# therealadityashankar/hey-buddy

Hardware: AMD Instinct MI355X
Metric: audio clips/sec featurized+trained, 1.5 s @16 kHz, 1/2/4/8 GPU (higher is better)
Workload: dtype f32

## Files before the change

### hey-buddy_amd/csrc/hbk_clip_ops.hip

```cpp
#include <algorithm>

#include "hbk_aug_dev.h"

namespace hbk {
namespace {

struct TanhArgs {
  const float* x;
  int64_t x_stride;
  float* out;
  int64_t out_stride;
  int64_t n_clips;
  const float* amount;
  const int32_t* idx;
  int64_t n_entries;
  SrcView view;
};

__device__ __forceinline__ unsigned abs_bits(float v, int s) {
  return s < kT ? (__builtin_bit_cast(unsigned, v) & 0x7FFFFFFFu) : 0xFFFFFFFFu;
}

__global__ void __launch_bounds__(kThreads) __attribute__((amdgpu_waves_per_eu(8)))
tanh_distortion_kernel(TanhArgs a) {
  __shared__ unsigned hist[4096];
  __shared__ float red[32];
  __shared__ unsigned pick[2];
  constexpr int kPer = (kT + kThreads - 1) / kThreads;
  const int64_t n_iter = a.idx ? a.n_entries : a.n_clips;
  for (int64_t e = blockIdx.x; e < n_iter; e += gridDim.x) {
    const int64_t clip = a.idx ? a.idx[e] : e;
    const int tid = opaque_tid();
    const float* x = a.x + clip * a.x_stride;
    float* out = a.out + clip * a.out_stride;
    const float amt = a.amount[clip];
    if (amt != amt) {
      if (out != x) copy_clip(x, out, tid);
      continue;
    }
    float xr[kPer];
    const int pre = a.view.pre ? a.view.pre[clip] : -1, len = a.view.pre ? a.view.len[clip] : 0;
    if (pre >= 0) {
      const int n = min(len, kT);
      const float* row = n > 0 ? a.view.src + clip * a.view.stride : x;
      const int t = opaque_tid();
      const int w0 = __builtin_amdgcn_readfirstlane(t & ~63);
#pragma unroll
      for (int u = 0; u < kPer; ++u) xr[u] = load_placed_wave(row, pre, n, w0 + u * kThreads, t & 63);
    } else {
    const int t = opaque_tid();
#pragma unroll
    for (int u = 0; u < kPer; ++u) {
      const int s = t + u * kThreads;
      xr[u] = s < kT ? *reinterpret_cast<const float*>(reinterpret_cast<const char*>(x) + (static_cast<uint32_t>(s) << 2))
                     : 0.f;
    }
    }
    const double pos = (100.0 - 99.0 * static_cast<double>(amt)) / 100.0 * (kT - 1);
    const int lo = min(max(static_cast<int>(floor(pos)), 0), kT - 1);
    const double frac = pos - lo;
    unsigned prefix = 0, mask = 0, rank = static_cast<unsigned>(lo);
#pragma unroll 1
    for (int p = 0; p < 3; ++p) {
      const int shift = p == 0 ? 19 : (p == 1 ? 9 : 0), bins = p == 0 ? 4096 : (p == 1 ? 1024 : 512);
      const int per_lane = bins >> 6;
      for (int i = tid; i < bins; i += kThreads) hist[i] = 0;
      __syncthreads();
      const int t = opaque_tid();
#pragma unroll
      for (int u = 0; u < kPer; ++u) {
        const unsigned b = abs_bits(xr[u], t + u * kThreads);
        if ((b & mask) == prefix && b != 0xFFFFFFFFu) atomicAdd(&hist[(b >> shift) & (bins - 1)], 1u);
      }
      __syncthreads();
      if (tid < 64) {
        unsigned own = 0;
        for (int i = 0; i < per_lane; ++i) own += hist[per_lane * tid + i];
        unsigned inc = own;
#pragma unroll
        for (int d = 1; d < 64; d <<= 1) {
          const unsigned v = __shfl_up(inc, d, 64);
          if (tid >= d) inc += v;
        }
        const unsigned long long hit = __ballot(inc > rank);
        const int l = __ffsll(static_cast<long long>(hit)) - 1;
        if (tid == l) {
          unsigned r = rank - (inc - own), dsel = per_lane * l;
          for (int i = 0; i < per_lane - 1; ++i) {
            const unsigned h = hist[dsel];
            if (r < h) break;
            r -= h;
            ++dsel;
          }
          pick[0] = dsel;
          pick[1] = r;
        }
      }
      __syncthreads();
      prefix |= pick[0] << shift;
      mask |= static_cast<unsigned>(bins - 1) << shift;
      rank = pick[1];
    }
    float cnt = 0.f, mg = __builtin_inff();
    const int t2 = opaque_tid();
#pragma unroll
    for (int u = 0; u < kPer; ++u) {
      const unsigned b = abs_bits(xr[u], t2 + u * kThreads);
      if (b == 0xFFFFFFFFu) continue;
      if (b <= prefix) cnt += 1.f;
      else mg = fminf(mg, __builtin_bit_cast(float, b));
    }
    cnt = block_sum(cnt, red);
    {
      for (int d = 32; d >= 1; d >>= 1) mg = fminf(mg, __shfl_xor(mg, d, 64));
      __syncthreads();
      if ((tid & 63) == 0) red[tid >> 6] = mg;
      __syncthreads();
      mg = red[0];
      for (int w = 1; w < kThreads / 64; ++w) mg = fminf(mg, red[w]);
    }
    const double v_lo = __builtin_bit_cast(float, prefix);
    const double v_hi = (cnt >= lo + 2 || lo + 1 >= kT) ? v_lo : static_cast<double>(mg);
    const double d = v_hi - v_lo;
    const double th = frac >= 0.5 ? v_hi - d * (1.0 - frac) : v_lo + d * frac;
    const float g = static_cast<float>(0.5 / (th + 1e-6));
    float ex = 0.f, ey = 0.f;
#pragma unroll
    for (int u = 0; u < kPer; ++u) {
      ex += xr[u] * xr[u];
      xr[u] = 1.f - __fdividef(2.f, __expf(2.f * g * xr[u]) + 1.f);
      ey += xr[u] * xr[u];
    }
    block_sum2(ex, ey, red);
    const float rms_x = sqrtf(ex / kT);
    const float post = rms_x > 1e-9f ? rms_x / sqrtf(ey / kT) : 1.f;
    const int t3 = opaque_tid();
#pragma unroll
    for (int u = 0; u < kPer; ++u) {
      const int s = t3 + u * kThreads;
      if (s < kT) *reinterpret_cast<float*>(reinterpret_cast<char*>(out) + (static_cast<uint32_t>(s) << 2)) = xr[u] * post;
    }
    __syncthreads();
  }
}

constexpr int kPlaceSpan = 4096;
__global__ void __launch_bounds__(256) place_kernel(const float* __restrict__ src, int64_t src_stride,
                                                    const int32_t* __restrict__ src_len,
                                                    const int32_t* __restrict__ pre,
                                                    const int32_t* __restrict__ idx, float* __restrict__ out,
                                                    int64_t out_stride, int64_t n_clips, int T) {
  const int spans = (T + kPlaceSpan - 1) / kPlaceSpan;
  const int64_t items = n_clips * spans;
  constexpr int kR = kPlaceSpan / 1024;
  for (int64_t it = blockIdx.x; it < items; it += gridDim.x) {
    const int64_t e = it / spans;
    const int sp = static_cast<int>(it - e * spans);
    const int64_t clip = idx ? idx[e] : e;
    const int p = pre[clip];
    const int n = min(src_len[clip], T);
    const int last = max(n - 1, 0);
    const float* s = src + clip * src_stride;
    float* o = out + clip * out_stride;
    const int t0 = sp * kPlaceSpan + 4 * static_cast<int>(threadIdx.x);
    float v[kR][4];
#pragma unroll
    for (int r = 0; r < kR; ++r)
#pragma unroll
      for (int q = 0; q < 4; ++q) {
        const int u = t0 + r * 1024 + q - p;
        const float x = n > 0 ? s[min(max(u, 0), last)] : 0.f;
        v[r][q] = (u >= 0 && u < n) ? x : 0.f;
      }
#pragma unroll
    for (int r = 0; r < kR; ++r) {
      const int t = t0 + r * 1024;
      if (t < T) *reinterpret_cast<float4*>(o + t) = make_float4(v[r][0], v[r][1], v[r][2], v[r][3]);
    }
  }
}

constexpr int kEqTile = 64;
struct EqArgs {
  const float* x;
  int64_t x_stride;
  const double* coef;
  const int32_t* idx;
  float* out;
  int64_t out_stride;
  int64_t n;
  SrcView view;
};

constexpr int kEqClips = 8;
__global__ void __launch_bounds__(64) eq_kernel(EqArgs a) {
  constexpr int kRow = kEqTile + 4;
  __shared__ __attribute__((aligned(16))) float tin[kEqClips][kRow];
  __shared__ __attribute__((aligned(16))) float tout[kEqClips][kRow];
  const int lane = threadIdx.x, c = lane >> 3, sec = lane & 7;
  const int64_t j0 = static_cast<int64_t>(blockIdx.x) * kEqClips;
  const int64_t jc = min(j0 + c, a.n - 1);
  const double* cf0 = a.coef + jc * 35;
  const bool copy = cf0[0] != cf0[0];
  const int k = min(sec, 6);
  double b0 = cf0[5 * k], b1 = cf0[5 * k + 1], b2 = cf0[5 * k + 2], a1 = cf0[5 * k + 3], a2 = cf0[5 * k + 4];
  if (copy) b0 = 1.0, b1 = b2 = a1 = a2 = 0.0;
  double s1 = 0.0, s2 = 0.0;
  const int lc = lane >> 3, lq = lane & 7;
  const int64_t jl = min(j0 + lc, a.n - 1);
  const int64_t clip_l = a.idx ? static_cast<int64_t>(a.idx[jl]) : jl;
  const float* xl = a.x + clip_l * a.x_stride;
  float* ol = a.out + clip_l * a.out_stride;
  const bool store_l = j0 + lc < a.n;
  const int pre_l = a.view.pre ? a.view.pre[clip_l] : -1, len_l = a.view.pre ? a.view.len[clip_l] : 0;
  const int n_l = pre_l >= 0 ? min(len_l, kT) : 0;
  const float* sl = n_l > 0 ? a.view.src + clip_l * a.view.stride : xl;
  float4 p0, p1;
  auto load_tile = [&](int t) {
    const int u0 = t + 4 * lq - pre_l;
    if (pre_l >= 0 && u0 >= 0 && u0 + 35 < n_l) {
      const float* q = sl + u0;
      p0 = float4{q[0], q[1], q[2], q[3]};
      p1 = float4{q[32], q[33], q[34], q[35]};
    } else if (pre_l >= 0 && (u0 + 35 < 0 || u0 >= n_l)) {
      p0 = p1 = float4{0.f, 0.f, 0.f, 0.f};
    } else if (pre_l >= 0) {
// ... 158 lines not shown
```

### hey-buddy_amd/csrc/hbk_embed.hip

```cpp
#include <algorithm>
#include <cmath>
#include <cstring>
#include <numeric>
#include <vector>

#include "hbk_common.h"
#include "hbk_embed_args.h"
#include "hbk_embed_plan.h"

namespace hbk {
namespace {

constexpr int kWaves = kThreads / 64;
constexpr int kChunkClips = 16384;
inline int64_t chunk_clips() {
  static const int64_t c = [] {
    const char* e = getenv("HBK_EMBED_CHUNK");
    const long long v = e ? atoll(e) : 0;
    return v >= 256 && v <= 32768 ? int64_t(v) : int64_t(kChunkClips);
  }();
  return c;
}

typedef float f4 __attribute__((ext_vector_type(4)));

template <int NB, int RB, bool WG>
__device__ __forceinline__ void conv_stage(const float* __restrict__ X, float* __restrict__ Y,
                                           const float* __restrict__ Wst,
                                           const int* __restrict__ ktab,
                                           const float* __restrict__ bias, int G, int hin, int win,
                                           const StageDesc& S, int wstride, int lane, int wave) {
  const int ho = hin - S.kh + 1, wo = win - S.kw + 1;
  const int img_pos = ho * wo, M = G * img_pos;
  const int nrb = (M + 15) >> 4;
  const int r16 = lane & 15, kq = lane >> 4;
  const int nblk = (S.cout + 15) >> 4;
  for (int cb = 0; cb < nblk; cb += NB)
  for (int rb0 = wave * RB; rb0 < nrb; rb0 += kWaves * RB) {
    int moff[RB];
#pragma unroll
    for (int r = 0; r < RB; ++r) {
      int m = min((rb0 + r) * 16 + r16, M - 1);
      const int g = m / img_pos;
      const int rem = m - g * img_pos;
      const int y = rem / wo;
      const int x = rem - y * wo;
      moff[r] = ((g * hin + y) * win + x) * S.cinp;
    }
    f4 acc[RB][NB];
#pragma unroll
    for (int r = 0; r < RB; ++r)
#pragma unroll
      for (int c = 0; c < NB; ++c) acc[r][c] = f4{0.f, 0.f, 0.f, 0.f};
    const float* wp = Wst + kq * wstride + cb * 16 + r16;
#pragma unroll 2
    for (int ks = 0; ks < S.ksteps; ++ks) {
      const int koff = ktab[ks * 4 + kq];
      float av[RB], bv[NB];
#pragma unroll
      for (int r = 0; r < RB; ++r) av[r] = X[moff[r] + koff];
#pragma unroll
      for (int c = 0; c < NB; ++c) bv[c] = wp[ks * 4 * wstride + min(c, nblk - 1 - cb) * 16];
#pragma unroll
      for (int r = 0; r < RB; ++r)
#pragma unroll
        for (int c = 0; c < NB; ++c)
          acc[r][c] = __builtin_amdgcn_mfma_f32_16x16x4f32(av[r], bv[c], acc[r][c], 0, 0, 0);
    }
#pragma unroll
    for (int c = 0; c < NB; ++c) {
      const int n = (cb + c) * 16 + r16;
      if (n >= S.cout) continue;
      const float bb = bias[n];
#pragma unroll
      for (int r = 0; r < RB; ++r)
#pragma unroll
        for (int i = 0; i < 4; ++i) {
          const int m = (rb0 + r) * 16 + kq * 4 + i;
          if (m < M) {
            float v = acc[r][c][i] + bb;
            if (S.act) v = v >= 0.f ? v : v * S.alpha;
            Y[m * S.coutp + n] = v;
          }
        }
    }
  }
  (void)WG;
}

template <int NB, int RB, bool WG>
__global__ void __launch_bounds__(kThreads) conv_chain_kernel(ChainArgs a) {
  extern __shared__ __attribute__((aligned(16))) float smem[];
  float* X = smem + a.lds_x;
  float* Y = smem + a.lds_y;
  float* Wl = smem + a.lds_w;
  int* ktab = reinterpret_cast<int*>(smem + a.lds_k);
  const int tid = threadIdx.x, lane = tid & 63, wave = tid >> 6;
  if (!WG)
    for (int i = tid; i < a.wblob_floats; i += kThreads) Wl[i] = a.wblob[i];

  const int64_t n_groups = (a.n_img + a.G - 1) / a.G;
  const int64_t n_tasks = n_groups * a.n_bands;
  const int C = a.C_src;
  const int cinp0 = a.st[0].cinp;
  for (int64_t task = blockIdx.x; task < n_tasks; task += gridDim.x) {
    const int64_t grp = task / a.n_bands;
    const int band = static_cast<int>(task - grp * a.n_bands);
    const int64_t img0 = grp * a.G;
    const int G = static_cast<int>(min<int64_t>(a.G, a.n_img - img0));
    const int orow0 = band * a.band;
    const int orows = min(a.band, a.H_out - orow0);
    const int r0 = orow0 * a.out_ph;
    const int rows_in = orows * a.out_ph + a.shrink;

    const int row_elems = a.W_in * C;
    const int per_img = rows_in * row_elems;
    for (int e = tid; e < G * per_img; e += kThreads) {
      const int g = e / per_img;
      int rem = e - g * per_img;
      const int r = rem / row_elems;
      rem -= r * row_elems;
      const int w = rem / C;
      const int c = rem - w * C;
      const int64_t im = img0 + g;
      const int64_t clip = im / a.ipc;
      const int roff = a.row_off[im - clip * a.ipc];
      const float* src = a.in + clip * a.src_clip_stride +
                         static_cast<int64_t>(roff + (r0 + r) * a.in_ph) * a.src_row_stride +
                         (w * a.in_pw) * C + c;
      float v = src[0];
      for (int i = 0; i < a.in_ph; ++i)
        for (int j = 0; j < a.in_pw; ++j) v = nan_max(v, src[i * a.src_row_stride + j * C]);
      X[((g * rows_in + r) * a.W_in + w) * cinp0 + c] = v;
    }

    int hin = rows_in, win = a.W_in;
    float* cur = X;
    float* nxt = Y;
    for (int s = 0; s < a.n_stages; ++s) {
      const StageDesc S = a.st[s];
      __syncthreads();
      for (int k = tid; k < S.ksteps * 4; k += kThreads) {
        int v = 0;
        if (k < S.K) {
          const int tap = k / S.cin;
          const int ci = k - tap * S.cin;
          const int dh = tap / S.kw;
          const int dw = tap - dh * S.kw;
          v = (dh * win + dw) * S.cinp + ci;
        }
        ktab[k] = v;
      }
      __syncthreads();
      const float* Wst = WG ? a.wblob + S.w_off : Wl + S.w_off;
      conv_stage<NB, RB, WG>(cur, nxt, Wst, ktab, a.wblob + S.b_off, G, hin, win, S, a.wstride,
                             lane, wave);
      float* t = cur;
      cur = nxt;
      nxt = t;
      hin -= S.kh - 1;
      win -= S.kw - 1;
    }
    __syncthreads();

    const int coutp = a.st[a.n_stages - 1].coutp;
    const int orow_elems = a.W_out * a.C_out;
    const int per_out = orows * orow_elems;
    for (int e = tid; e < G * per_out; e += kThreads) {
      const int g = e / per_out;
      int rem = e - g * per_out;
      const int r = rem / orow_elems;
      rem -= r * orow_elems;
      const int w = rem / a.C_out;
      const int c = rem - w * a.C_out;
      const float* p = cur + ((g * hin + r * a.out_ph) * win + w * a.out_pw) * coutp + c;
// ... 1892 lines not shown
    case Kern::p1s: return f ? addr(p1s_chain_kernel<true>) : addr(p1s_chain_kernel<false>);
    case Kern::p2s: return f ? addr(p2s_chain_kernel<true>) : addr(p2s_chain_kernel<false>);
    case Kern::t3s: return f ? addr(t3s_chain_kernel<true>) : addr(t3s_chain_kernel<false>);
  }
  return nullptr;
}

hipError_t set_max_dynamic_lds(const void* fn) {
  hipFuncAttributes at;
  hipError_t e = hipFuncGetAttributes(&at, fn);
  if (e != hipSuccess) return e;
  return hipFuncSetAttribute(fn, hipFuncAttributeMaxDynamicSharedMemorySize,
                             int(160 * 1024 - static_cast<int>(at.sharedSizeBytes)));
}

void set_pointers(ChainArgs& a, const Launch&, const unsigned char* blob) {
  a.wblob = reinterpret_cast<const float*>(blob);
}
void set_pointers(XArgs& x, const Launch& L, const unsigned char* blob) {
  x.wblob = reinterpret_cast<const _Float16*>(blob);
  x.bblob = reinterpret_cast<const float*>(blob + L.ptr_off[1]);
  x.ktab = reinterpret_cast<const int*>(blob + L.ptr_off[2]);
  x.i2c_off = reinterpret_cast<const int*>(blob + L.ptr_off[3]);
}
template <class A>
void set_pointers(A& p, const Launch& L, const unsigned char* blob) {
  p.w = reinterpret_cast<const _Float16*>(blob);
  if (L.ptr_off[1] >= L.blob.size()) return;
  const float* bias = reinterpret_cast<const float*>(blob + L.ptr_off[1]);
  if constexpr (std::is_same_v<A, P2sArgs>) p.bias_a = bias;
  else p.bias = bias;
}

int realise(const Launch& L, bool pattern, bool debug, Slot& s) {
  const void* fn = kernel_address(L.kernel);
  hipError_t e = hipMalloc(&s.d_blob, L.blob.size());
  if (e != hipSuccess && !pattern) return hip_error(e, "hipMalloc chain weights");
  if (e == hipSuccess) e = hipMemcpy(s.d_blob, L.blob.data(), L.blob.size(), hipMemcpyHostToDevice);
  if (e != hipSuccess && !pattern) return hip_error(e, "copy chain weights");
  if (pattern) {
    if (e == hipSuccess) e = hipFuncSetAttribute(fn, hipFuncAttributeMaxDynamicSharedMemorySize, int(L.lds_bytes));
    if (e == hipSuccess) e = hipOccupancyMaxActiveBlocksPerMultiprocessor(&s.blocks_per_cu, fn, L.threads, L.lds_bytes);
    if (e != hipSuccess || s.blocks_per_cu < 1) {
      (void)hipGetLastError();
      if (s.d_blob) (void)hipFree(s.d_blob);
      s.d_blob = nullptr;
      return HBK_OK;
    }
  } else {
    if (L.lds_bytes > 64 * 1024) {
      e = set_max_dynamic_lds(fn);
      if (e != hipSuccess) return hip_error(e, "hipFuncSetAttribute(max dynamic LDS)");
    }
    s.blocks_per_cu = L.kernel.kind == Kern::exact
                          ? 2
                          : std::max<int>(1, std::min<int>(4, int((160 * 1024) / std::max<size_t>(L.lds_bytes, 1))));
  }
  s.plan = &L;
  s.fn = fn;
  s.args = L.args;
  std::visit([&](auto& a) { set_pointers(a, L, static_cast<const unsigned char*>(s.d_blob)); }, s.args);
  if (debug && pattern) fprintf(stderr, "%s, %d blocks/CU\n", L.debug.c_str(), s.blocks_per_cu);
  if (debug && !pattern) fputs(L.debug.c_str(), stderr);
  return HBK_OK;
}

int realise_program(const ProgramPlan& prog, bool debug, std::vector<ChainPlan>& dev) {
  dev.resize(prog.chains.size());
  for (size_t k = 0; k < dev.size(); ++k) {
    const int rc = realise(prog.chains[k].base, false, debug, dev[k].base);
    if (rc) return rc;
    if (prog.chains[k].pattern) realise(*prog.chains[k].pattern, true, debug, dev[k].pattern);
  }
  return HBK_OK;
}

void bind(ChainArgs& a, const float* in, int64_t stride, float* out, int64_t n_img, int*) {
  a.in = in;
  a.src_clip_stride = stride;
  a.out = out;
  a.n_img = n_img;
}
void bind(XArgs& x, const float* in, int64_t stride, float* out, int64_t n_img, int* range_flag) {
  x.range_flag = range_flag;
  x.in = in;
  x.src_clip_stride = stride;
  x.out = out;
  if ((reinterpret_cast<uintptr_t>(x.out) & 15) || (x.out_img_stride & 3)) x.vec_out = 0;
  if ((reinterpret_cast<uintptr_t>(x.in) & 15) || (x.src_clip_stride & 3) || (x.src_row_stride & 3)) x.raw_vec = 0;
  x.n_img = n_img;
}
template <class A>
void bind(A& p, const float* in, int64_t stride, float* out, int64_t n_img, int* range_flag) {
  p.range_flag = range_flag;
  p.in = in;
  if constexpr (std::is_same_v<A, T3sArgs>) p.src_clip_stride = stride;
  else p.src_img_stride = stride;
  p.out = out;
  p.n_img = n_img;
}

int run_program(const ProgramPlan& prog, const std::vector<ChainPlan>& dev, const int* d_gather, const float* in,
                int64_t n_units, int64_t in_unit_stride, float* out, int64_t out_unit_floats, float* ws,
                int64_t chunk, hipStream_t stream, int* range_flag, int k_begin = 0, int k_end = -1) {
  const int n_ch = static_cast<int>(prog.chains.size());
  if (k_end < 0) k_end = n_ch;
  for (int64_t u0 = 0; u0 < n_units; u0 += chunk) {
    const int64_t nu = std::min(chunk, n_units - u0);
    float* bufs[2] = {ws, ws + chunk * prog.buf_floats[0]};
    for (int k = k_begin; k < k_end; ++k) {
      const ChainHost& h = prog.chains[k];
      const int src_buf = (k == k_begin && k_begin > 0) ? -1 : h.src_buf;
      const int dst_buf = (k == k_end - 1 && k_end < n_ch) ? -1 : h.dst_buf;
      const float* src = src_buf < 0 ? in + u0 * in_unit_stride : bufs[src_buf];
      const int64_t stride = src_buf < 0 ? in_unit_stride : h.src_clip_stride;
      float* dst = dst_buf < 0 ? out + u0 * out_unit_floats : bufs[dst_buf];
      const int64_t n_img = nu * h.imgs_per_unit;
      for (const Slot* s : {&dev[k].pattern, &dev[k].base}) {
        if (!s->fn) continue;
        const Launch& L = *s->plan;
        if (s == &dev[k].pattern) {
          const bool aligned = !(reinterpret_cast<uintptr_t>(src) & 15) && !(stride & 3) &&
                               !(reinterpret_cast<uintptr_t>(dst) & 15) && !(L.out_stride_4 & 3);
          if (!aligned || stride < L.min_src_stride) continue;
          if (L.tasks_below_2_31 && n_img * L.n_bands >= (int64_t(1) << 31)) continue;
        }
        KernelArgs args = s->args;
        void* argp = std::visit(
            [&](auto& a) -> void* {
              bind(a, src, stride, dst, n_img, range_flag);
              return &a;
            },
            args);
        const int64_t tasks = ((n_img + L.imgs_per_task - 1) / L.imgs_per_task) * L.n_bands;
        const int64_t blocks = std::min<int64_t>(tasks, persistent_blocks(s->blocks_per_cu, stream));
        if (blocks > 0) {
          (void)hipLaunchKernel(s->fn, dim3(unsigned(blocks)), dim3(L.threads), &argp, L.lds_bytes, stream);
          HBK_LAUNCH_CHECK(L.name);
        }
        break;
      }
    }
    if (prog.gather_buf >= 0 && k_end == n_ch) {
      const int n_out = static_cast<int>(prog.gather_src.size());
      const int row = static_cast<int>(out_unit_floats / n_out);
      hipLaunchKernelGGL(embed_gather_kernel, dim3(unsigned((nu + 3) / 4)), dim3(256), 0, stream,
                         bufs[prog.gather_buf], out + u0 * out_unit_floats, d_gather, nu, prog.n_src, n_out, row);
      HBK_LAUNCH_CHECK("embed_gather_kernel");
    }
  }
  return HBK_OK;
}

int run_units(const hbk_embed_plan* p, bool clips, const float* in, int64_t n, int64_t in_stride, int64_t min_stride,
              float* out, int64_t out_floats, void* workspace, int64_t workspace_bytes, void* stream, int k_begin = 0,
              int k_end = -1) {
  if (n < 0) return arg_error(clips ? "negative n_clips" : "negative n");
  if (n == 0) return HBK_OK;
  if (!in || !out || !workspace) return arg_error("NULL pointer");
  if (in_stride < min_stride) return arg_error("mel_clip_stride < seq_frames * in_w");
  int64_t need = 0;
  hbk_embed_workspace_size(p, n, &need);
  if (workspace_bytes < need) return arg_error("workspace too small");
  return run_program(clips ? p->host.clip : p->host.win, clips ? p->clip : p->win, p->d_gather, in, n, in_stride, out,
                     out_floats, static_cast<float*>(workspace), std::min<int64_t>(n, chunk_clips()),
                     as_stream(stream), p->d_range, k_begin, k_end);
}

}
}

extern "C" {

int hbk_embed_plan_create(const hbk_graph_op* ops, int32_t n_ops, int32_t in_h, int32_t in_w,
                          const int32_t* win_start, int32_t n_win, hbk_embed_plan** plan) {
  return hbk_embed_plan_create_ex(ops, n_ops, in_h, in_w, win_start, n_win, HBK_PREC_SPLIT_F16, plan);
}

int hbk_embed_plan_create_ex(const hbk_graph_op* ops, int32_t n_ops, int32_t in_h, int32_t in_w,
                             const int32_t* win_start, int32_t n_win, int32_t precision,
                             hbk_embed_plan** plan) {
  using namespace hbk;
  if (!plan) return arg_error("plan is NULL");
  *plan = nullptr;
  if (precision != HBK_PREC_SPLIT_F16 && precision != HBK_PREC_EXACT_F32) return arg_error("unknown precision");
  if (!ops || n_ops <= 0) return arg_error("empty graph");
  if (in_h <= 0 || in_w <= 0) return arg_error("bad window size");
  if (!win_start || n_win <= 0 || n_win > kMaxWin) return arg_error("n_win must be in [1, 32]");
  auto* p = new hbk_embed_plan();
  auto fail = [&](int rc) {
    hbk_embed_plan_destroy(p);
    return rc;
  };
  const EmbedKnobs knobs = read_embed_knobs();
  std::vector<OpIn> graph;
  for (int i = 0; i < n_ops; ++i) {
    const hbk_graph_op& o = ops[i];
    graph.push_back(OpIn{o.kind, o.kh, o.kw, o.cin, o.cout, o.act, o.alpha, o.weight, o.bias});
  }
  int rc = plan_embed(graph, in_h, in_w, std::vector<int>(win_start, win_start + n_win),
                      precision == HBK_PREC_SPLIT_F16, knobs, p->host);
  if (rc) {
    set_error("%s", p->host.error.c_str());
    return fail(rc);
  }
  hipError_t e = hipMalloc(reinterpret_cast<void**>(&p->d_range), sizeof(int));
  if (e == hipSuccess) e = hipMemset(p->d_range, 0, sizeof(int));
  if (e != hipSuccess) return fail(hip_error(e, "hipMalloc range flag"));
  rc = realise_program(p->host.clip, knobs.debug, p->clip);
  if (rc) return fail(rc);
  if (const std::vector<int>& map = p->host.clip.gather_src; !map.empty()) {
    e = hipMalloc(reinterpret_cast<void**>(&p->d_gather), map.size() * sizeof(int));
    if (e == hipSuccess) e = hipMemcpy(p->d_gather, map.data(), map.size() * sizeof(int), hipMemcpyHostToDevice);
    if (e != hipSuccess) return fail(hip_error(e, "embed gather map"));
    if (knobs.debug) fputs(p->host.dedup_debug.c_str(), stderr);
  }
  rc = realise_program(p->host.win, knobs.debug, p->win);
  if (rc) return fail(rc);
  *plan = p;
  return HBK_OK;
}

int hbk_embed_plan_destroy(hbk_embed_plan* p) {
  if (!p) return HBK_OK;
  for (auto* dev : {&p->clip, &p->win})
    for (auto& c : *dev)
      for (hbk::Slot* s : {&c.pattern, &c.base})
        if (s->d_blob) (void)hipFree(s->d_blob);
  if (p->d_gather) (void)hipFree(p->d_gather);
  if (p->d_range) (void)hipFree(p->d_range);
  delete p;
  return HBK_OK;
}

int hbk_embed_plan_info(const hbk_embed_plan* p, int32_t* out_dim, int32_t* n_prefix_ops,
                        int32_t* n_chains, double* prefix_macs, double* tail_macs,
                        int32_t* seq_frames) {
  if (!p) return hbk::arg_error("plan is NULL");
  if (out_dim) *out_dim = p->host.out_dim;
  if (n_prefix_ops) *n_prefix_ops = p->host.n_prefix;
  if (n_chains) *n_chains = static_cast<int32_t>(p->host.clip.chains.size());
  if (prefix_macs) *prefix_macs = p->host.prefix_macs;
  if (tail_macs) *tail_macs = p->host.tail_macs;
  if (seq_frames) *seq_frames = p->host.seq_frames;
  return HBK_OK;
}

}

namespace hbk {

constexpr int kNanBlocks = 2048;
constexpr int kNanPatchBlocks = 512;

__global__ void __launch_bounds__(256) nan_flags_kernel(const float* __restrict__ rows, int64_t n, int64_t row_len,
                                                        int64_t per, int32_t* __restrict__ flags,
                                                        int32_t* __restrict__ blk_good, int32_t* __restrict__ bad,
                                                        int32_t* __restrict__ meta) {
  __shared__ int32_t s_good;
  if (threadIdx.x == 0) s_good = 0;
  __syncthreads();
  const int lane = threadIdx.x & 63, wave = threadIdx.x >> 6;
  const int64_t lo = static_cast<int64_t>(blockIdx.x) * per, hi = min<int64_t>(n, lo + per);
  int32_t n_good = 0;
  for (int64_t r = lo + wave; r < hi; r += 4) {
    const float4* p = reinterpret_cast<const float4*>(rows + r * row_len);
    bool nan = false;
    for (int64_t j = lane; j < row_len / 4; j += 64) {
      const float4 v = p[j];
      nan |= (v.x != v.x) | (v.y != v.y) | (v.z != v.z) | (v.w != v.w);
    }
    const bool any = __ballot(nan) != 0;
    if (lane == 0) {
      flags[r] = any ? 1 : 0;
      if (any)
        bad[atomicAdd(meta, 1)] = static_cast<int32_t>(r);
      else
        ++n_good;
    }
  }
  if (lane == 0) atomicAdd(&s_good, n_good);
  __syncthreads();
  if (threadIdx.x == 0) blk_good[blockIdx.x] = s_good;
}

__global__ void __launch_bounds__(256) nan_list_kernel(int64_t n, int64_t per, const int32_t* __restrict__ flags,
                                                       const int32_t* __restrict__ blk_good,
                                                       int32_t* __restrict__ good, const int32_t* __restrict__ meta) {
  __shared__ int32_t s_w[4];
  __shared__ int32_t s_off;
  if (meta[0] == 0) return;
  const int tid = threadIdx.x, lane = tid & 63, wave = tid >> 6;
  int32_t off = 0;
  for (int i = tid; i < static_cast<int>(blockIdx.x); i += 256) off += blk_good[i];
  for (int o = 32; o > 0; o >>= 1) off += __shfl_xor(off, o, 64);
  if (lane == 0) s_w[wave] = off;
  __syncthreads();
  if (tid == 0) s_off = s_w[0] + s_w[1] + s_w[2] + s_w[3];
  __syncthreads();
  off = s_off;
  const int64_t lo = static_cast<int64_t>(blockIdx.x) * per, hi = min<int64_t>(n, lo + per);
  for (int64_t base = lo; base < hi; base += 256) {
    const int64_t r = base + tid;
    const bool keep = r < hi && flags[r] == 0;
    const uint64_t m = __ballot(keep);
    const int32_t below = __popcll(m & ((uint64_t(1) << lane) - 1));
    __syncthreads();
    if (lane == 0) s_w[wave] = __popcll(m);
    __syncthreads();
    int32_t pre = 0;
    for (int w = 0; w < wave; ++w) pre += s_w[w];
    if (keep) good[off + pre + below] = static_cast<int32_t>(r);
    off += s_w[0] + s_w[1] + s_w[2] + s_w[3];
  }
}

__device__ __forceinline__ uint64_t nan_hash(uint64_t z) {
  z = (z ^ (z >> 30)) * 0xBF58476D1CE4E5B9ull;
  z = (z ^ (z >> 27)) * 0x94D049BB133111EBull;
  return z ^ (z >> 31);
}

__global__ void __launch_bounds__(256) nan_patch_kernel(float* __restrict__ rows, int64_t n, int64_t row_len,
                                                        const int32_t* __restrict__ bad,
                                                        const int32_t* __restrict__ good,
                                                        const int32_t* __restrict__ meta, uint64_t seed) {
  const int64_t n_bad = meta[0];
  if (n_bad == 0) return;
  const int64_t n_good = n - n_bad;
  const int lane = threadIdx.x & 63;
  const int64_t nw = static_cast<int64_t>(gridDim.x) * 4;
  for (int64_t i = (static_cast<int64_t>(blockIdx.x) * 256 + threadIdx.x) >> 6; i < n_bad; i += nw) {
    const int64_t r = bad[i];
    float4* dst = reinterpret_cast<float4*>(rows + r * row_len);
    if (n_good == 0) {
      for (int64_t j = lane; j < row_len / 4; j += 64) dst[j] = float4{0.f, 0.f, 0.f, 0.f};
      continue;
    }
    const uint64_t h = nan_hash(seed ^ (0x9E3779B97F4A7C15ull * static_cast<uint64_t>(r + 1)));
    const int64_t src = good[static_cast<int64_t>((static_cast<unsigned __int128>(h) * static_cast<uint64_t>(n_good)) >> 64)];
    const float4* sp = reinterpret_cast<const float4*>(rows + src * row_len);
    for (int64_t j = lane; j < row_len / 4; j += 64) dst[j] = sp[j];
  }
}

}

extern "C" {

int hbk_embed_workspace_size(const hbk_embed_plan* p, int64_t n, int64_t* bytes) {
  using namespace hbk;
  if (!p || !bytes) return arg_error("plan/bytes is NULL");
  if (n < 0) return arg_error("negative n");
  const int64_t chunk = std::max<int64_t>(1, std::min<int64_t>(n, chunk_clips()));
  const int64_t *bc = p->host.clip.buf_floats, *bw = p->host.win.buf_floats;
  *bytes = chunk * std::max(bc[0] + bc[1], bw[0] + bw[1]) * int64_t(sizeof(float)) + 256;
  return HBK_OK;
}

int hbk_embed_clips(const hbk_embed_plan* p, const float* mel, int64_t n_clips, int64_t mel_clip_stride,
                    float* out, void* workspace, int64_t workspace_bytes, void* stream) {
  using namespace hbk;
  if (!p) return arg_error("plan is NULL");
  return run_units(p, true, mel, n_clips, mel_clip_stride, int64_t(p->host.seq_frames) * p->host.in_w, out,
                   int64_t(p->host.n_win) * p->host.out_dim, workspace, workspace_bytes, stream);
}

int hbk_embed_split_info(const hbk_embed_plan* p, int32_t n_front, int64_t* mid_floats_per_clip) {
  using namespace hbk;
  if (!p || !mid_floats_per_clip) return arg_error("plan/mid_floats_per_clip is NULL");
  const int n = static_cast<int>(p->host.clip.chains.size());
  if (n_front < 1 || n_front >= n) return arg_error("n_front must be in [1, n_chains - 1]");
  const ChainHost& c = p->host.clip.chains[n_front - 1];
  *mid_floats_per_clip = c.out_img_stride * c.imgs_per_unit;
  return HBK_OK;
}

int hbk_embed_clips_front(const hbk_embed_plan* p, const float* mel, int64_t n_clips, int64_t mel_clip_stride,
                          int32_t n_front, float* mid, void* workspace, int64_t workspace_bytes, void* stream) {
  using namespace hbk;
  int64_t mid_floats = 0;
  int rc = hbk_embed_split_info(p, n_front, &mid_floats);
  if (rc) return rc;
  return run_units(p, true, mel, n_clips, mel_clip_stride, int64_t(p->host.seq_frames) * p->host.in_w, mid,
                   mid_floats, workspace, workspace_bytes, stream, 0, n_front);
}

int hbk_embed_clips_back(const hbk_embed_plan* p, const float* mid, int64_t n_clips, int32_t n_front, float* out,
                         void* workspace, int64_t workspace_bytes, void* stream) {
  using namespace hbk;
  int64_t mid_floats = 0;
  int rc = hbk_embed_split_info(p, n_front, &mid_floats);
  if (rc) return rc;
  return run_units(p, true, mid, n_clips, mid_floats, 0, out, int64_t(p->host.n_win) * p->host.out_dim, workspace,
                   workspace_bytes, stream, n_front, -1);
}

int hbk_embed_windows(const hbk_embed_plan* p, const float* windows, int64_t n, float* out,
                      void* workspace, int64_t workspace_bytes, void* stream) {
  using namespace hbk;
  if (!p) return arg_error("plan is NULL");
  return run_units(p, false, windows, n, int64_t(p->host.in_h) * p->host.in_w, 0, out, p->host.out_dim, workspace,
                   workspace_bytes, stream);
}

int64_t hbk_nan_rows_workspace_size(int64_t n) {
  return n < 0 ? 0 : (3 * n + hbk::kNanBlocks + 1) * int64_t(sizeof(int32_t));
}

int hbk_nan_rows_fix(float* rows, int64_t n, int64_t row_len, uint64_t seed, void* workspace,
                     int64_t workspace_bytes, void* stream) {
  using namespace hbk;
  if (n < 0 || row_len <= 0 || row_len % 4) return arg_error("n >= 0, row_len a positive multiple of 4");
  if (n == 0) return HBK_OK;
  if (n >= (int64_t(1) << 31)) return arg_error("n >= 2^31 rows");
  if (!rows || !workspace) return arg_error("NULL pointer");
  if ((reinterpret_cast<uintptr_t>(rows) & 15)) return arg_error("rows must be 16-B aligned");
  if (workspace_bytes < hbk_nan_rows_workspace_size(n)) return arg_error("workspace too small");
  int32_t* flags = static_cast<int32_t*>(workspace);
  int32_t* good = flags + n;
  int32_t* bad = good + n;
  int32_t* blk_good = bad + n;
  int32_t* meta = blk_good + kNanBlocks;
  hipStream_t st = as_stream(stream);
  hipError_t e = hipMemsetAsync(meta, 0, sizeof(int32_t), st);
  if (e != hipSuccess) return hip_error(e, "hbk_nan_rows_fix");
  const int64_t blocks = std::min<int64_t>(kNanBlocks, (n + 3) / 4);
  const int64_t per = (n + blocks - 1) / blocks;
  const int64_t used = (n + per - 1) / per;
  hipLaunchKernelGGL(nan_flags_kernel, dim3(unsigned(used)), dim3(256), 0, st, rows, n, row_len, per, flags,
                     blk_good, bad, meta);
  HBK_LAUNCH_CHECK("nan_flags_kernel");
  hipLaunchKernelGGL(nan_list_kernel, dim3(unsigned(used)), dim3(256), 0, st, n, per, flags, blk_good, good, meta);
  HBK_LAUNCH_CHECK("nan_list_kernel");
  const int64_t pblocks = std::min<int64_t>(kNanPatchBlocks, (n + 3) / 4);
  hipLaunchKernelGGL(nan_patch_kernel, dim3(unsigned(pblocks)), dim3(256), 0, st, rows, n, row_len, bad, good, meta,
                     seed);
  HBK_LAUNCH_CHECK("nan_patch_kernel");
  return HBK_OK;
}

int hbk_embed_range_status(const hbk_embed_plan* p, int32_t* tripped, int32_t reset, void* stream) {
  using namespace hbk;
  if (!p || !tripped) return arg_error("plan/tripped is NULL");
  int32_t h = 0;
  hipError_t e = hipMemcpyAsync(&h, p->d_range, sizeof(int32_t), hipMemcpyDeviceToHost, as_stream(stream));
  if (e == hipSuccess) e = hipStreamSynchronize(as_stream(stream));
  if (e == hipSuccess && reset && h) e = hipMemsetAsync(p->d_range, 0, sizeof(int32_t), as_stream(stream));
  if (e != hipSuccess) return hip_error(e, "hbk_embed_range_status");
  *tripped = h;
  return HBK_OK;
}

}

#ifdef HBK_PHASE_TIMING
extern "C" int hbk_debug_phase_cycles(unsigned long long* out, int n) {
  unsigned long long h[64];
  if (hipMemcpyFromSymbol(h, HIP_SYMBOL(hbk::g_phase_cycles), sizeof(h)) != hipSuccess) return -2;
  for (int i = 0; i < n && i < 64; ++i) out[i] = h[i];
  unsigned long long z[64] = {};
  (void)hipMemcpyToSymbol(HIP_SYMBOL(hbk::g_phase_cycles), z, sizeof(z));
  return 0;
}
#endif

#ifdef HBK_TRACE
extern "C" int hbk_debug_trace(unsigned long long* out, int* counts) {
  if (hipMemcpyFromSymbol(out, HIP_SYMBOL(hbk::g_trace), sizeof(unsigned long long) * 4 * 4 * 256) != hipSuccess)
    return -2;
  if (hipMemcpyFromSymbol(counts, HIP_SYMBOL(hbk::g_trace_n), sizeof(int) * 16) != hipSuccess) return -2;
  int z[16] = {};
  (void)hipMemcpyToSymbol(HIP_SYMBOL(hbk::g_trace_n), z, sizeof(z));
  return 0;
}
#endif
```

### hey-buddy_amd/csrc/hbk_embed_plan.h

```cpp
#pragma once

#include <algorithm>
#include <cmath>
#include <cstdarg>
#include <cstdio>
#include <cstring>
#include <initializer_list>
#include <numeric>
#include <optional>
#include <string>
#include <variant>
#include <vector>

#include "hbk_embed_args.h"

namespace hbk {
namespace {

constexpr int kPlanOk = 0, kPlanErrArg = -1, kPlanErrUnsupported = -3;
constexpr int kOpConv = 0, kOpMaxPool = 1;

struct EmbedKnobs {
  bool lds_kb_set = false;
  int lds_kb = 0;
// ... 832 lines not shown
inline void assign_buffers(ProgramPlan& prog, bool clip_path, int n_win) {
  const size_t n = prog.chains.size();
  bool tail = false;
  int tail_imgs = n_win;
  for (size_t k = 0; k < n; ++k) {
    ChainHost& c = prog.chains[k];
    c.src_buf = (k == 0) ? -1 : int((k - 1) % 2);
    c.dst_buf = (k + 1 == n && prog.gather_src.empty()) ? -1 : int(k % 2);
    if (clip_path && c.ipc > 1 && !tail) {
      tail = true;
      tail_imgs = c.ipc;
    }
    c.imgs_per_unit = tail ? tail_imgs : 1;
    if (c.dst_buf >= 0)
      prog.buf_floats[c.dst_buf] = std::max(prog.buf_floats[c.dst_buf], c.out_img_stride * c.imgs_per_unit);
  }
  if (!prog.gather_src.empty()) prog.gather_buf = int((n - 1) % 2);
}

inline int plan_embed(const std::vector<OpIn>& graph, int in_h, int in_w, const std::vector<int>& starts,
                      bool split_f16, const EmbedKnobs& knobs, EmbedHostPlan& p) {
  std::string& err = p.error;
  const int n_ops = static_cast<int>(graph.size()), n_win = static_cast<int>(starts.size());
  p.in_h = in_h;
  p.in_w = in_w;
  p.n_win = n_win;
  p.split_f16 = split_f16;
  for (int s : starts)
    if (s < 0) return arg_fail(err, "negative window start");
  std::vector<OpInfo> ops;
  Dims d{in_h, in_w, 1};
  std::vector<Dims> dims;
  for (int i = 0; i < n_ops; ++i) {
    const OpIn& o = graph[i];
    OpInfo op{o.kind, o.kh, o.kw, o.cin, o.cout, o.act, o.alpha, {}, {}};
    if (o.kh <= 0 || o.kw <= 0) return arg_fail(err, "kernel / pool size must be positive");
    if (o.kind == kOpConv) {
      if (o.cin != d.c || o.cout <= 0 || !o.weight || !o.bias) return arg_fail(err, "bad conv op");
      op.w.assign(o.weight, o.weight + size_t(o.kh) * o.kw * o.cin * o.cout);
      op.b.assign(o.bias, o.bias + o.cout);
      if (split_f16)
        for (float w : op.w)
          if (!(std::fabs(w) < kF16Max)) {
            err = strf("hbk: op %d has a weight |w| >= 65504 (or NaN), outside the split-f16 range; "
                       "use HBK_PREC_EXACT_F32", i);
            return kPlanErrUnsupported;
          }
      d = Dims{d.h - o.kh + 1, d.w - o.kw + 1, o.cout};
    } else if (o.kind == kOpMaxPool) {
      d = Dims{d.h / o.kh, d.w / o.kw, d.c};
    } else {
      return arg_fail(err, "unknown op kind");
    }
    if (d.h <= 0 || d.w <= 0) return arg_fail(err, "graph collapses the window");
    ops.push_back(std::move(op));
    dims.push_back(d);
  }
  if (d.h != 1 || d.w != 1) return arg_fail(err, "graph output must be 1 x 1 x C");
  p.out_dim = d.c;

  int g = 0;
  for (int s : starts) g = std::gcd(g, s);
  int stride = 1, split = n_ops, last_pool = -1, stride_before_last = 1;
  for (int i = 0; i < n_ops; ++i) {
    if (ops[i].kind == kOpMaxPool) {
      const int ns = stride * ops[i].kh;
      if (g % ns != 0) {
        split = i;
        break;
      }
      last_pool = i;
      stride_before_last = stride;
      stride = ns;
    }
  }
  if (split == n_ops && last_pool > 0) {
    split = last_pool;
    stride = stride_before_last;
  }
  if (split == n_ops || split == 0) {
    err = "hbk: graph has no window-splitting pool; use hbk_embed_windows";
    return kPlanErrUnsupported;
  }
  p.n_prefix = split;
  p.split_stride = stride;
  p.seq_frames = *std::max_element(starts.begin(), starts.end()) + in_h;

  int rc;
  {
    std::vector<Dims> od;
    rc = plan_segment(ops, 0, split, Dims{p.seq_frames, in_w, 1}, 1, {0}, 0, in_w, split_f16, knobs, p.clip, &od, err);
    if (rc) return rc;
    const Dims pre = od.back();
    const Dims wd = dims[split - 1];
    std::vector<int> roff;
    for (int s : starts) roff.push_back(s / stride);
    for (int r : roff)
      if (r + wd.h > pre.h) return arg_fail(err, "window start beyond the frame sequence");
    const size_t n_pre = p.clip.chains.size();
    std::vector<int> phases, win_src;
    int H = 0;
    {
      int S = 1;
      for (int i = split; i < n_ops; ++i)
        if (ops[i].kind == kOpMaxPool) S *= ops[i].kh;
      for (int r : roff)
        if (std::find(phases.begin(), phases.end(), r % S) == phases.end()) phases.push_back(r % S);
      std::sort(phases.begin(), phases.end());
      for (int r : roff) H = std::max(H, r - r % S + wd.h);
      bool ok = S > 1 && !knobs.no_dedup && int(phases.size()) < n_win;
      for (int ph : phases) ok = ok && ph + H <= pre.h;
      Dims t{H, wd.w, wd.c};
      for (int i = split; i < n_ops && ok; ++i) {
        const OpInfo& o = ops[i];
        t = o.kind == kOpConv ? Dims{t.h - o.kh + 1, t.w - o.kw + 1, o.cout} : Dims{t.h / o.kh, t.w / o.kw, t.c};
        ok = t.h > 0 && t.w > 0;
      }
      ok = ok && t.w == 1 && int(phases.size()) * t.h <= n_win;
      if (ok) {
        for (int r : roff) {
          const int ph = int(std::find(phases.begin(), phases.end(), r % S) - phases.begin());
          const int row = (r - r % S) / S;
          ok = ok && row < t.h;
          win_src.push_back(ph * t.h + row);
        }
        p.clip.n_src = int(phases.size()) * t.h;
      }
      if (!ok) phases.clear();
    }
    const int64_t pre_floats = int64_t(pre.h) * pre.w * pre.c;
    if (!phases.empty()) {
      p.clip.gather_src = win_src;
      rc = plan_segment(ops, split, n_ops, Dims{H, wd.w, wd.c}, int(phases.size()), phases, pre_floats,
                        pre.w * pre.c, split_f16, knobs, p.clip, nullptr, err);
      p.dedup_debug = strf("hbk tail dedup: %zu phase images of %d rows per clip for %d windows\n", phases.size(), H,
                           n_win);
    } else {
      rc = plan_segment(ops, split, n_ops, Dims{wd.h, wd.w, wd.c}, n_win, roff, pre_floats, pre.w * pre.c, split_f16,
                        knobs, p.clip, nullptr, err);
    }
    if (rc) return rc;
    for (size_t k = 0; k < p.clip.chains.size(); ++k)
      (k < n_pre ? p.prefix_macs : p.tail_macs) += p.clip.chains[k].macs_per_img;
    if (!phases.empty()) p.tail_macs *= double(phases.size()) / double(n_win);
    assign_buffers(p.clip, true, n_win);
  }
  rc = plan_segment(ops, 0, n_ops, Dims{in_h, in_w, 1}, 1, {0}, int64_t(in_h) * in_w, in_w, split_f16, knobs, p.win,
                    nullptr, err);
  if (rc) return rc;
  assign_buffers(p.win, false, 1);
  return kPlanOk;
}

}
}
```

Baseline: 1.131 million.

## Size embed chunks to persistent-kernel rounds and aggregate zero-bin histogram counts

The embed chunk size, previously fixed at 16384 clips, is now derived from how many images each persistent kernel processes per launch round. The chunk becomes a small multiple (2–4) of the LCM of those round sizes, so each chunk holds whole rounds and the last one has no partial tail. Separately, the tanh distortion radix-select histogram now counts hits in bin 0 with a wave ballot and popcount, then adds them with one atomic per wave, to reduce LDS atomic contention on a bin that many elements may fall into. Smaller chunks mean more launches per batch and a little more host-side planning work.

```diff
diff --git a/hey-buddy_amd/csrc/hbk_clip_ops.hip b/hey-buddy_amd/csrc/hbk_clip_ops.hip
--- a/hey-buddy_amd/csrc/hbk_clip_ops.hip
+++ b/hey-buddy_amd/csrc/hbk_clip_ops.hip
@@ -67,11 +67,16 @@
       for (int i = tid; i < bins; i += kThreads) hist[i] = 0;
       __syncthreads();
       const int t = opaque_tid();
+      unsigned n0 = 0;
 #pragma unroll
       for (int u = 0; u < kPer; ++u) {
         const unsigned b = abs_bits(xr[u], t + u * kThreads);
-        if ((b & mask) == prefix && b != 0xFFFFFFFFu) atomicAdd(&hist[(b >> shift) & (bins - 1)], 1u);
-      }
+        const unsigned dg = (b >> shift) & (bins - 1);
+        const bool in = (b & mask) == prefix && b != 0xFFFFFFFFu;
+        n0 += static_cast<unsigned>(__popcll(__ballot(in && dg == 0)));
+        if (in && dg != 0) atomicAdd(&hist[dg], 1u);
+      }
+      if ((t & 63) == 0 && n0 != 0) atomicAdd(&hist[0], n0);
       __syncthreads();
       if (tid < 64) {
         unsigned own = 0;
diff --git a/hey-buddy_amd/csrc/hbk_embed.hip b/hey-buddy_amd/csrc/hbk_embed.hip
--- a/hey-buddy_amd/csrc/hbk_embed.hip
+++ b/hey-buddy_amd/csrc/hbk_embed.hip
@@ -12,15 +12,15 @@
 namespace {
 
 constexpr int kWaves = kThreads / 64;
-constexpr int kChunkClips = 16384;
-inline int64_t chunk_clips() {
+inline int64_t chunk_forced() {
   static const int64_t c = [] {
     const char* e = getenv("HBK_EMBED_CHUNK");
     const long long v = e ? atoll(e) : 0;
-    return v >= 256 && v <= 32768 ? int64_t(v) : int64_t(kChunkClips);
+    return v >= kEmbedChunkForcedMin && v <= kEmbedChunkForcedMax ? int64_t(v) : int64_t(0);
   }();
   return c;
 }
+inline int64_t chunk_cap() { return chunk_forced() ? chunk_forced() : int64_t(kEmbedChunkCap); }
 
 typedef float f4 __attribute__((ext_vector_type(4)));
 
@@ -2219,6 +2219,21 @@
   return HBK_OK;
 }
 
+int64_t chunk_clips(const ProgramPlan& prog, const std::vector<ChainPlan>& dev, int k_begin, int k_end,
+                    hipStream_t stream) {
+  const int n_ch = static_cast<int>(prog.chains.size());
+  if (k_end < 0) k_end = n_ch;
+  int64_t round = 0;
+  for (int k = std::max(k_begin, 0); k < std::min(k_end, n_ch); ++k) {
+    const Slot& s = dev[k].pattern;
+    if (!s.fn || (s.plan->kernel.kind != Kern::p0s && s.plan->kernel.kind != Kern::p1s)) continue;
+    const int64_t imgs = persistent_blocks(s.blocks_per_cu, stream) * s.plan->imgs_per_task;
+    const int64_t per_unit = std::max<int64_t>(1, prog.chains[k].imgs_per_unit);
+    if (imgs % per_unit == 0) round = embed_round_join(round, imgs / per_unit);
+  }
+  return std::min(chunk_cap(), embed_chunk_clips(round, chunk_forced()));
+}
+
 int run_units(const hbk_embed_plan* p, bool clips, const float* in, int64_t n, int64_t in_stride, int64_t min_stride,
               float* out, int64_t out_floats, void* workspace, int64_t workspace_bytes, void* stream, int k_begin = 0,
               int k_end = -1) {
@@ -2229,8 +2244,10 @@
   int64_t need = 0;
   hbk_embed_workspace_size(p, n, &need);
   if (workspace_bytes < need) return arg_error("workspace too small");
-  return run_program(clips ? p->host.clip : p->host.win, clips ? p->clip : p->win, p->d_gather, in, n, in_stride, out,
-                     out_floats, static_cast<float*>(workspace), std::min<int64_t>(n, chunk_clips()),
+  const ProgramPlan& prog = clips ? p->host.clip : p->host.win;
+  const std::vector<ChainPlan>& dev = clips ? p->clip : p->win;
+  const int64_t chunk = std::min<int64_t>(n, chunk_clips(prog, dev, k_begin, k_end, as_stream(stream)));
+  return run_program(prog, dev, p->d_gather, in, n, in_stride, out, out_floats, static_cast<float*>(workspace), chunk,
                      as_stream(stream), p->d_range, k_begin, k_end);
 }
 
@@ -2419,7 +2436,7 @@
   using namespace hbk;
   if (!p || !bytes) return arg_error("plan/bytes is NULL");
   if (n < 0) return arg_error("negative n");
-  const int64_t chunk = std::max<int64_t>(1, std::min<int64_t>(n, chunk_clips()));
+  const int64_t chunk = std::max<int64_t>(1, std::min<int64_t>(n, chunk_cap()));
   const int64_t *bc = p->host.clip.buf_floats, *bw = p->host.win.buf_floats;
   *bytes = chunk * std::max(bc[0] + bc[1], bw[0] + bw[1]) * int64_t(sizeof(float)) + 256;
   return HBK_OK;
diff --git a/hey-buddy_amd/csrc/hbk_embed_plan.h b/hey-buddy_amd/csrc/hbk_embed_plan.h
--- a/hey-buddy_amd/csrc/hbk_embed_plan.h
+++ b/hey-buddy_amd/csrc/hbk_embed_plan.h
@@ -1008,5 +1008,21 @@
   return kPlanOk;
 }
 
-}
-}
+constexpr int kEmbedChunkCap = 16384, kEmbedChunkTarget = 3072;
+constexpr int kEmbedChunkMinRounds = 2, kEmbedChunkMaxRounds = 4;
+constexpr int kEmbedChunkForcedMin = 256, kEmbedChunkForcedMax = 32768;
+inline int64_t embed_chunk_clips(int64_t round_clips, int64_t forced) {
+  if (forced >= kEmbedChunkForcedMin && forced <= kEmbedChunkForcedMax) return forced;
+  if (round_clips <= 0 || round_clips > kEmbedChunkCap) return kEmbedChunkCap;
+  const int64_t fit = std::min<int64_t>(kEmbedChunkMaxRounds, kEmbedChunkTarget / round_clips);
+  const int64_t rounds = std::max<int64_t>(kEmbedChunkMinRounds, fit);
+  return std::min(rounds, kEmbedChunkCap / round_clips) * round_clips;
+}
+inline int64_t embed_round_join(int64_t r0, int64_t r1) {
+  if (r0 <= 0 || r1 <= 0) return std::max<int64_t>(0, std::max(r0, r1));
+  if (r0 > kEmbedChunkCap || r1 > kEmbedChunkCap) return int64_t(kEmbedChunkCap) + 1;
+  return std::lcm(r0, r1);
+}
+
+}
+}
```

Measured after the change: 1.148 million (median of 6 runs). 1.5% higher.
